# JohannesBuchner/UltraNest

Hardware: AMD Instinct MI355X
Metric: proposal-points filtered/sec (MLFriends.inside) + region-rebuild ms, N=4000 d=50 (higher is better)
Workload: dtype f64; 1 GPU; C5: N=4000 live points, d=50, P=1e6 proposals/step/GPU drawn uniformly inside the wrapping ellipsoid (set E), AffineLayer, 30 bootstraps; one step = MLFriends.inside on a batch resident in HBM; the timed loop visits 3 distinct batches in turn; n_live=4000, d=50, bootstraps=30, parallelism=proposal rows sharded over 1 GPU(s), region replicated

## Files before the change

### ultranest_amd/csrc/mlf_debug.hip

```cpp
#include <hip/hip_runtime.h>

#include <atomic>
#include <vector>

#include "../../include/mlfriends_hip.h"
#include "mlf_host.hpp"
#include "mlf_sample.hpp"

using namespace mlf;

extern "C" {

int mlf_debug_forget_grants(unsigned long long *grants_so_far) {
  if (grants_so_far) *grants_so_far = g_grant_calls.load(std::memory_order_relaxed);
  g_grant_epoch.fetch_add(1u, std::memory_order_acq_rel);
  return 0;
}

int mlf_debug_philox(uint64_t seed, unsigned stream, size_t nblocks, uint32_t *out) {
  if (!out) return fail_arg(MLF_E_BADARG, "null pointer");
  if (nblocks == 0) return 0;
  if (int rc = ensure_ctx()) return rc;
  Ctx &c = g_ctx;
  CK(c.out.reserve(nblocks * 4 * sizeof(unsigned)));
// ... 108 lines not shown
  }
  if (f.segcnt.p && f.segcnt.cap >= sizeof(unsigned)) {
    const size_t n = (size_t)f.last.nsegs;
    std::vector<unsigned> c(n);
    if (n) CK(hipMemcpy(c.data(), f.segcnt.p, n * sizeof(unsigned), hipMemcpyDeviceToHost));
    unsigned long long sum = 0, mx = 0;
    for (unsigned v : c) {
      sum += v;
      mx = v > mx ? v : mx;
    }
    out[2] = sum;
    out[3] = mx;
    out[4] = n;
  }
  if (f.png.p) {
    unsigned g[6];
    CK(hipMemcpy(g, f.png.p, sizeof g, hipMemcpyDeviceToHost));
    out[5] = g[0];
    if (cap > 6) out[6] = g[1];
    if (cap > 7) out[7] = g[5];
  }
  if (cap > 17) {
    out[16] = (unsigned long long)f.last_min.cut[0];
    out[17] = (unsigned long long)f.last_min.cut[1];
  }
  if (cap > 18) out[18] = (f.last_min.defer && (f.last_min.fused_variant & 2u)) ? 1ull : 0ull;
  {
    if (cap >= 16 && f.last.mid && f.last.time_launches && f.segcnt.p) {
      unsigned st[8];
      CK(hipMemcpy(st, f.segcnt.p, sizeof st, hipMemcpyDeviceToHost));
      for (int i = 0; i < 8; ++i) out[8 + i] = st[i];
    } else if (cap >= 16 && f.last.nsegs == uncertain_blocks() && f.segcnt.cap >= (size_t)(f.last.nsegs + 8) * sizeof(unsigned)) {
      unsigned st[8];
      CK(hipMemcpy(st, f.segcnt.as<unsigned>() + uncertain_stamp_base(), sizeof st, hipMemcpyDeviceToHost));
      for (int i = 0; i < 8; ++i) out[8 + i] = st[i];
    }
  }
  return 0;
}
// ... 50 lines not shown
```

### ultranest_amd/csrc/mlf_filter.hpp

```cpp
#pragma once
#include "mlf_common.hpp"
#include "mlf_prep4.hpp"

#define MLF_FILTER_MAXD 128

constexpr int kFilterMaxSplit = 16;

namespace mlf {

struct FilterArgs {
  const void *refF;
  const void *qF;
  const float *tlo, *thi;
  int ntiles32;
  long long ngroups;
  long long nq;
  int *best;
  unsigned long long *list;
  unsigned seg_cap;
  unsigned *seg_count;
  unsigned *counters;
  int tile0, tile1;
  const int *qmap;
  const unsigned *ngroups_dev;
// ... 16 lines not shown
  const void *qF;
  const float *tlo, *thi;
  const int *qmap;
  const int *qmin;
  long long ngroups;
  const unsigned *nslots_dev;
  long long nq;
  int *best;
  void *cq;
  float *ctlo, *cthi;
  int *cmap;
  int *cmin;
  unsigned *ccount;
  unsigned ccap;
  int last;
  unsigned long long *stamps;
  unsigned stamp_block;
};
constexpr unsigned kUncertainListCap = 4096;
struct UncertainArgs {
  const void *refF;
  int ntiles32;
  const void *qF;
  const float *thi;
  const int *qmap;
  const unsigned *nslots_dev;
  const double *pts;
  int d, dp;
  const double *lay_ctr;
  const double *T8;
  int ldt8;
  const double *refR;
  int n;
  double r2;
  int *best;
  unsigned *counters;
  unsigned *seg_count;
  EllExactArgs ell;
  unsigned nsweepblk;
};
hipError_t launch_sweep_min(int ks, int qw, const MinArgs &a, hipStream_t s);
// ... 94 lines not shown
```

### ultranest_amd/csrc/mlf_fused.hip

```cpp
#include "mlf_filter.hpp"
#include "mlf_dpp_dev.hpp"
#include "mlf_filter_dev.hpp"
#include "mlf_prep4.hpp"

#include <math.h>

namespace mlf {

typedef float float16v __attribute__((ext_vector_type(16)));
typedef _Float16 half2v __attribute__((ext_vector_type(2)));
typedef _Float16 half8v __attribute__((ext_vector_type(8)));
typedef float float2v __attribute__((ext_vector_type(2)));
typedef unsigned uint4v __attribute__((ext_vector_type(4)));

#ifndef MLF_OPERAND_STEPS
#define MLF_OPERAND_STEPS 4
#endif
namespace {

template <int DP, int NW = 8>
struct F4 {
  static constexpr int NS = (DP + 15) / 16;
  static constexpr int KS = (DP + 6 + 15) / 16;
  static constexpr int NT = (KS + 1) / 2;
// ... 551 lines not shown
      if ((keepm[g] >> row) & 1u) {
        const unsigned rank = base + (unsigned)__popc(keepm[g] & ((1u << row) - 1u));
        const size_t gd = rank >> 5;
        const unsigned rd = (rank & 31u) + (unsigned)(lane & 32);
        if (rank < a.ccap) {
#pragma unroll
          for (int s = 0; s < KS; ++s) {
            union { half8v h8; uint4 u; } cv;
            cv.h8 = bq[g][s];
            dst[(gd * KS + s) * 64 + rd] = cv.u;
          }
        }
        if (lane < 32 && rank < a.ccap) {
          a.ctlo[rank] = tlo[g];
          a.cthi[rank] = thi[g];
          a.cmap[rank] = (int)((g0 + g) * 32 + p32);
          a.cmin[rank] = qmn[g];
        }
      }
      base += (unsigned)__popc(keepm[g]);
    }
  }
  stamp(12);
}

bool fused_usable(int dp) { return dp >= 2 && dp <= 56 && (dp & 1) == 0; }

template <int D, int NW, bool SQ>
static hipError_t launch_prep_sweep_t(const FusedArgs &a, long long nsets, hipStream_t s) {
  constexpr size_t lds = F4<D, NW>::LDS;
  static_assert(lds <= 160 * 1024 - 64, "LDS budget");
// ... 32 lines not shown
```

### ultranest_amd/csrc/mlf_recheck_dev.hpp

```cpp
#pragma once
#include "mlf_prep4.hpp"

namespace mlf {

constexpr unsigned kEllWaves = 512;

__device__ __forceinline__ void ell_exact_wave(const EllExactArgs &a, double *dls, unsigned wave, unsigned nwaves) {
  const unsigned count = *a.count < a.cap ? *a.count : a.cap;
  const int lane = threadIdx.x & 63;
  const int d = a.d;
  const bool own = lane < d;
  const double *lcol = a.ell_L + (own ? lane : 0);
  const double myctr = own ? a.ell_ctr[lane] : 0.0;
  for (unsigned e = wave; e < count; e += nwaves) {
    const long long p = a.list[e];
    const double *row = a.pts + p * (long long)d;
    const double dl = own ? row[lane] - myctr : 0.0;
    __builtin_amdgcn_wave_barrier();
    dls[lane] = dl;
    __builtin_amdgcn_wave_barrier();
    double y = 0.0;
#pragma unroll 10
    for (int j = 0; j < d; ++j) y = __builtin_fma(lcol[(size_t)j * a.dp], dls[j], y);
    if (!own) y = 0.0;
    double qt = y * y, nrm2 = dl * dl;
    for (int o = 32; o > 0; o >>= 1) {
      qt += __shfl_xor(qt, o, 64);
      nrm2 += __shfl_xor(nrm2, o, 64);
    }
    const double eps = a.eps_scale * nrm2;
    bool inside;
    if (a.chol_ok && qt + eps < a.enlarge) {
      inside = true;
    } else if (a.chol_ok && qt - eps > a.enlarge) {
      inside = false;
    } else {
      double acc = 0.0;
      if (lane == 0) {
        for (int j = 0; j < d; ++j) {
          const double dj = row[j] - a.ell_ctr[j];
          const double *arow = a.ell_A + (size_t)j * a.dp;
          for (int k = 0; k < d; ++k) acc += (dj * arow[k]) * (row[k] - a.ell_ctr[k]);
        }
      }
      acc = __shfl(acc, 0, 64);
      inside = acc <= a.enlarge;
    }
    if (!inside && lane == 0) {
      a.gate[p] = 0;
      if (a.route) a.route[p] = 0;
    }
  }
  if (lane == 0) {
    const unsigned t = atomicAdd(a.done, 1u);
    if (t == nwaves - 1u) {
      if (a.last) *a.last = *a.count;
      *a.count = 0u;
      *a.done = 0u;
    }
  }
}

constexpr int kTQ = 8;
constexpr int kChunk = 32;

// ... 104 lines not shown
```

### ultranest_amd/csrc/mlf_route.hip

```cpp
#include <hip/hip_runtime.h>

#include <algorithm>

#include "../../include/mlfriends_hip.h"
#include "mlf_host.hpp"
#include "mlf_prep3.hpp"
#include "mlf_prep64.hpp"

namespace mlf {

int filter_prepare_refs(FilterCtx &f, const double *refR, int n, int d, int dp, hipStream_t s,
                        bool host_sync) {
  f.refs_ready = false;
  const int ks = (dp + 6 + 15) / 16;
  if (ks > 9 || n < 1 || (long long)round_up(n, 32) / 32 * ks * 1024 >= (1ll << 31)) {
    f.usable = false;
    return 0;
  }
  f.ks = ks;
  const int npad32 = round_up(n, 32);
  f.ntiles32 = npad32 / 32;
  CK(f.stats.reserve((8 + MLF_FILTER_MAXD) * sizeof(double)));
  CK(f.refF.reserve((size_t)npad32 * ks * 16 * 2));
  (void)d;
// ... 86 lines not shown
  if (!p.filter) return p;
  p.ordered = !first_index && f.ordered && opt(f, OPT_ORDER);
  const bool bounded = p.stage == STAGE_PREP4;
  p.mid = bounded && !pregate && !first_index && f.ks <= 4 && mid_usable(r->dp) && nq <= opt(f, OPT_MID_MAX);
  if (p.mid) return p;
  const int want_phases = (int)opt(f, OPT_PHASES);
  const long long phase_min = opt(f, OPT_PHASE_MIN_QUERIES);
  if (want_phases && nq >= phase_min && (phase_min < 32768 || nq * f.ntiles32 >= 30000000ll))
    p.nphase = want_phases >= 2 ? (want_phases <= f.ntiles32 / 4 ? want_phases : (f.ntiles32 >= 16 ? 2 : 1))
                                : (f.ntiles32 >= 16 ? 2 : 1);
  p.narrow = (p.nphase > 1 && f.ks <= 4) ? (int)opt(f, OPT_NARROW_TAIL) : 0;
  const long long ngroups = (nq + 31) / 32;
  p.split = p.nphase == 1 ? filter_tile_split(f.ks, ngroups, f.ntiles32, (int)opt(f, OPT_SPLIT_WAVES)) : 1;
  p.own_recheck = bounded && !first_index && p.nphase == 1;
  p.fold_finish = bounded && p.nphase == 2;
  p.min_path = p.fold_finish && !first_index && f.ks <= 4 && opt(f, OPT_SWEEP_MIN);
  if (p.nphase == 2) {
    const int nt = f.ntiles32, first_pct = (int)opt(f, OPT_FIRST_RANGE_PCT), second_pct = (int)opt(f, OPT_SECOND_RANGE_PCT);
    const int cut = (int)((long long)nt * first_pct / 100);
    p.cut[0] = cut < 4 ? 4 : (cut > nt - 4 ? nt - 4 : cut);
    if (p.min_path && second_pct > 0 && nq * nt >= opt(f, OPT_THIRD_MIN_WORK)) {
      const int cut2 = (int)((long long)nt * second_pct / 100);
      int a = (int)((long long)cut2 * first_pct / 100);
      a = a < 4 ? 4 : a;
      if (cut2 >= a + 4 && cut2 <= nt - 4) {
        p.cut[0] = a;
        p.cut[1] = cut2;
      }
    }
  }
  p.defer = p.min_path && opt(f, OPT_FUSED_FIRST) && fused_usable(r->dp);
// ... 81 lines not shown
  FilterCtx &f = b.f;
  const BatchPlan &p = b.p;
  const ExactSrc &xs = *b.xs;
  const long long nqpad = b.ngroups() * 32;
  const bool min3 = p.cut[1] > 0;
  CK(f.segcnt.reserve((size_t)(p.nsegs + 8) * sizeof(unsigned)));
  CK(f.pmin.reserve((size_t)nqpad * sizeof(int)));
  if (min3) CK(f.pmin2.reserve((size_t)nqpad * sizeof(int)));
  MinArgs m{};
  m.refF = b.opF();
  m.ntiles32 = f.ntiles32;
  m.nq = b.nq;
  m.best = f.best.as<int>();
  m.ngroups = b.ngroups();
  m.ccap = (unsigned)nqpad;
  m.tile0 = 0;
  m.tile1 = p.cut[0];
  m.qF = f.qF.p;
  m.tlo = f.tlo.as<float>();
  m.thi = f.thi.as<float>();
  m.cq = f.pqF[0].p;
  m.ctlo = f.ptlo[0].as<float>();
  m.cthi = f.pthi[0].as<float>();
  m.cmap = f.pmap[0].as<int>();
  m.cmin = f.pmin.as<int>();
  m.ccount = f.png.as<unsigned>() + 2;
  m.last = 0;
  if (p.defer) {
    FusedArgs fu{};
    fu.p = xs.prep;
    fu.refF = b.opF();
    fu.ntiles32 = f.ntiles32;
    fu.tile0 = 0;
    fu.tile1 = p.cut[0];
    fu.cq = m.cq;
    fu.ctlo = m.ctlo;
    fu.cthi = m.cthi;
    fu.cmap = m.cmap;
    fu.cmin = m.cmin;
    fu.ccount = m.ccount;
    fu.ccap = m.ccap;
    if (f.stamp_block >= 0 && f.stamp_block < 1000000) {
// ... 9 lines not shown
  }
  const int usrc = min3 ? 0 : 1;
  m.tile0 = p.cut[0];
  m.tile1 = min3 ? p.cut[1] : f.ntiles32;
  m.qF = f.pqF[0].p;
  m.tlo = f.ptlo[0].as<float>();
  m.thi = f.pthi[0].as<float>();
  m.qmap = f.pmap[0].as<int>();
  m.qmin = f.pmin.as<int>();
  m.nslots_dev = f.png.as<unsigned>() + 2;
  m.cq = f.pqF[1].p;
  m.ctlo = f.ptlo[1].as<float>();
  m.cthi = f.pthi[1].as<float>();
  m.cmap = f.pmap[1].as<int>();
  m.cmin = min3 ? f.pmin2.as<int>() : nullptr;
  m.ccount = f.png.as<unsigned>() + 3;
  m.last = min3 ? 0 : 1;
  auto sweep_stamps = [&](int which) -> int {
    m.stamps = nullptr;
    if (f.stamp_block >= which * 1000000 && f.stamp_block < (which + 1) * 1000000) {
      CK(f.fstamps.reserve(16 * sizeof(unsigned long long)));
      m.stamps = f.fstamps.as<unsigned long long>();
      m.stamp_block = (unsigned)(f.stamp_block - which * 1000000);
    }
    return 0;
  };
  if (int rc = sweep_stamps(1)) return rc;
  if (min3) {
    if (int rc = timed_launch(b, [&] { return launch_sweep_min(f.ks, filter_groups_per_wave(f.ks, 0), m, b.s); })) return rc;
    if (int rc = sweep_stamps(2)) return rc;
    m.tile0 = p.cut[1];
    m.tile1 = f.ntiles32;
    m.qF = f.pqF[1].p;
    m.tlo = f.ptlo[1].as<float>();
    m.thi = f.pthi[1].as<float>();
    m.qmap = f.pmap[1].as<int>();
    m.qmin = f.pmin2.as<int>();
    m.nslots_dev = f.png.as<unsigned>() + 3;
    m.cq = f.pqF[0].p;
    m.ctlo = f.ptlo[0].as<float>();
    m.cthi = f.pthi[0].as<float>();
    m.cmap = f.pmap[0].as<int>();
    m.cmin = nullptr;
    m.ccount = f.png.as<unsigned>() + 4;
    m.last = 1;
  }
  if (int rc = timed_launch(b, [&] { return launch_sweep_min(f.ks, filter_groups_per_wave(f.ks, 0), m, b.s); })) return rc;
  UncertainArgs ua{};
  ua.refF = b.opF();
  ua.ntiles32 = f.ntiles32;
  ua.qF = f.pqF[usrc].p;
  ua.thi = f.pthi[usrc].as<float>();
  ua.qmap = f.pmap[usrc].as<int>();
  ua.nslots_dev = f.png.as<unsigned>() + (min3 ? 4 : 3);
  ua.pts = xs.pts;
  ua.d = b.L.d;
  ua.dp = b.L.dp;
  ua.lay_ctr = xs.lay_ctr;
  ua.T8 = xs.T8;
  ua.ldt8 = xs.ldt;
  ua.refR = b.opR();
  ua.n = b.L.n;
  ua.r2 = b.L.r2;
  ua.best = f.best.as<int>();
  ua.counters = f.counters.as<unsigned>();
  ua.seg_count = f.segcnt.as<unsigned>();
  ua.ell = xs.ell;
  if (int rc = timed_launch(b, [&] { return launch_uncertain(f.ks, ua, b.s); })) return rc;
  if (b.ev_after) CK(hipEventRecord(b.ev_after, b.s));
// ... 120 lines not shown
  const int mode = b.out_idx ? SCAN_FIRST : SCAN_MASK;
  if (!b.xs)
    launch_filter_finalize(f.route.as<uint8_t>(), f.best.as<int>(), f.counters.as<unsigned>(), b.nq, b.out_mask,
                           b.out_idx, f.gate2.as<uint8_t>(), b.s);
  ScanArgs a = b.xs ? scan_args(b.L, b.xs->pts, b.L.d, 1, b.nq, mode) : scan_args(b.L, b.q, b.ldq, b.ldk, b.nq, mode);
  a.gate = f.gate2.as<uint8_t>();
  a.out_idx = b.out_idx;
  a.out_mask = b.out_mask;
  a.only_gated = 1;
  if (b.xs) {
    scan_finalise(a, f, *b.xs);
    a.fin_best = f.best.as<int>();
    if (p.fold_finish) {
      a.fin_slots = f.png.as<unsigned>() + 2;
      a.fin_groups = f.png.as<unsigned>();
      if (p.min_path) a.fin_slots2 = f.png.as<unsigned>() + (p.cut[1] > 0 ? 4 : 3);
      if (p.cut[1] > 0) a.fin_slots3 = f.png.as<unsigned>() + 3;
    }
  }
  CK(launch_scan(b.L.dp, a, b.s));
  CK(hipGetLastError());
  return 0;
}

}

int filter_run(const FilterBatch &b) {
  FilterCtx &f = b.f;
  const BatchPlan &p = b.p;
  const long long nqpad = b.ngroups() * 32;
  f.last = p;
  if (p.min_path) f.last_min = p;
  if (int rc = filter_reserve(f, p, b.nq)) return rc;
  if (p.stage != STAGE_PREP4 && p.stage != STAGE_PREP3)
    launch_quant_queries(b.q, b.ldq, b.nq, nqpad, b.L.d, b.L.dp, f.ks, f.stats.as<double>(), b.L.r2, b.gate, f.qF.p,
                         f.tlo.as<float>(), f.thi.as<float>(), f.route.as<uint8_t>(), f.best.as<int>(),
                         f.counters.as<unsigned>(), b.s);
  CK(hipGetLastError());
  if (p.nphase > 1) {
    for (int i = 0; i < 2; ++i) {
      CK(f.pqF[i].reserve((size_t)nqpad * f.ks * 16 * 2));
      CK(f.ptlo[i].reserve((size_t)nqpad * sizeof(float)));
      CK(f.pthi[i].reserve((size_t)nqpad * sizeof(float)));
      CK(f.pmap[i].reserve((size_t)nqpad * sizeof(int)));
    }
    if (!f.png.p) {
      CK(f.png.reserve(8 * sizeof(unsigned)));
      CK(hipMemset(f.png.p, 0, 8 * sizeof(unsigned)));
    } else if (f.png_dirty) {
      CK(hipMemsetAsync(f.png.p, 0, 8 * sizeof(unsigned), b.s));
    }
    f.png_dirty = true;
  }
  if (int rc = p.min_path ? filter_sweep_min(b) : filter_phases(b)) return rc;
  if (!p.min_path && !p.own_recheck)
    if (int rc = filter_recheck(b)) return rc;
  if (int rc = filter_scan_tail(b)) return rc;
  if (p.nphase > 1) f.png_dirty = false;
  return 0;
}

}
```

### ultranest_amd/csrc/mlf_scan.hip

```cpp
#include "mlf_common.hpp"

namespace mlf {

template <int DP, int QB, bool EXTRA>
__global__ __launch_bounds__(kScanThreads) void k_scan(ScanArgs a) {
  constexpr int kScanQB = QB;
  __shared__ __attribute__((aligned(16))) double qs[kScanQB * DP];
  __shared__ int state[kScanQB];
  __shared__ int cnt[kScanQB];

  const int tid = threadIdx.x;
  const int lane = tid & 63;
  const int wave = tid >> 6;
  __shared__ int any_active;
  if (EXTRA && a.fin_best && blockIdx.x >= a.fin_grid0) {
    const long long p0 = (((long long)blockIdx.x - a.fin_grid0) * kScanThreads + tid) * 4;
    if (p0 == 0 && a.fin_reset) *a.fin_reset = 0u;
    if (p0 == 0 && a.fin_slots) {
      *a.fin_groups = (*a.fin_slots + 31u) / 32u;
      *a.fin_slots = 0u;
    }
    if (p0 == 0 && a.fin_slots2) {
      a.fin_groups[1] = *a.fin_slots2;
      *a.fin_slots2 = 0u;
    }
    if (p0 == 0 && a.fin_slots3) {
      a.fin_groups[5] = (*a.fin_slots3 + 31u) / 32u;
      *a.fin_slots3 = 0u;
    } else if (p0 == 0 && a.fin_slots2) {
      a.fin_groups[5] = 0u;
    }
    if (p0 >= a.nq) return;
    const bool overflowed = a.counters[1] != 0u;
    int rt[4], b[4];
    if (p0 + 3 < a.nq) {
      const uchar4 r4 = *reinterpret_cast<const uchar4 *>(a.route + p0);
      const int4 b4 = *reinterpret_cast<const int4 *>(a.fin_best + p0);
      rt[0] = r4.x, rt[1] = r4.y, rt[2] = r4.z, rt[3] = r4.w;
      b[0] = b4.x, b[1] = b4.y, b[2] = b4.z, b[3] = b4.w;
// ... 190 lines not shown
```

### ultranest_amd/csrc/mlf_sweepmin.hip

```cpp
#include "mlf_filter.hpp"
#include "mlf_dpp_dev.hpp"
#include "mlf_filter_dev.hpp"
#include "mlf_recheck_dev.hpp"

#include <math.h>

namespace mlf {

typedef __attribute__((ext_vector_type(8))) _Float16 half8;
typedef __attribute__((ext_vector_type(16))) float float16v;
typedef __attribute__((ext_vector_type(4))) unsigned uint4v;

namespace {

__device__ __forceinline__ int min3i(int a, int b, int c) {
  const int m = a < b ? a : b;
  return m < c ? m : c;
}

constexpr int kPosInf = 0x7f800000;

template <int KS>
__device__ __forceinline__ void load_tile(half8 (&A)[KS], __amdgpu_buffer_rsrc_t rsrc, int voff, int soff) {
#pragma unroll
// ... 37 lines not shown

constexpr int min_waves(int ks, int qw, int pf) {
  const int need = 16 * qw + 4 * ks * qw + 4 * ks * (pf + 1) + 40;
  return (qw <= 2 && ks * qw <= 8) ? 4 : (need <= 128 ? 4 : (need <= 168 ? 3 : 2));
}

constexpr long long kSweepMinSetGrid = 1024;

}

template <int KS, int QW, int PF>
__global__ __launch_bounds__(256) __attribute__((amdgpu_waves_per_eu(min_waves(KS, QW, PF)))) void k_sweep_min(MinArgs a) {
  const int lane = threadIdx.x & 63;
  const long long nslots = a.nslots_dev ? (long long)*a.nslots_dev : -1;
  const long long ngroups = nslots >= 0 ? (nslots + 31) / 32 : a.ngroups;
  __shared__ unsigned wg_keep[4], wg_base;
  bool stamp_on = a.stamps != nullptr && blockIdx.x == a.stamp_block && threadIdx.x < 64;
  auto stamp = [&](int k) __attribute__((always_inline)) {
    if (stamp_on) {
      const unsigned long long t = __builtin_readcyclecounter();
      if (lane == 0) a.stamps[k] = t;
    }
  };
  stamp(0);
  auto stamp_rt = [&](int k) __attribute__((always_inline)) {
    if (a.stamps != nullptr && threadIdx.x == 0) {
      if (blockIdx.x == 0) a.stamps[8 + k] = __builtin_amdgcn_s_memrealtime();
      if (blockIdx.x == a.stamp_block) a.stamps[10 + k] = __builtin_amdgcn_s_memrealtime();
    }
  };
  stamp_rt(0);
  for (unsigned bidx = blockIdx.x, pass = 0;; bidx += gridDim.x, ++pass) {
  if ((long long)bidx * (4 * QW) >= ngroups) break;
  if (pass) __syncthreads();
  const long long wave = (long long)bidx * 4 + (threadIdx.x >> 6);
  const long long g0 = wave * QW;
  if (g0 >= ngroups) {
    if (lane == 0) wg_keep[threadIdx.x >> 6] = 0u;
    __syncthreads();
    __syncthreads();
    continue;
  }

  const half8 *qF = reinterpret_cast<const half8 *>(a.qF);
  half8 bq[QW][KS];
  float tlo[QW], thi[QW];
  int run[QW], qnum[QW];
#pragma unroll
  for (int g = 0; g < QW; ++g) {
    const long long grp = (g0 + g < ngroups) ? g0 + g : ngroups - 1;
#pragma unroll
    for (int s = 0; s < KS; ++s) bq[g][s] = qF[((size_t)grp * KS + s) * 64 + lane];
    const long long qi = grp * 32 + (lane & 31);
    const bool have = g0 + g < ngroups && (nslots < 0 || qi < nslots);
    tlo[g] = have ? a.tlo[qi] : -1.0f;
    thi[g] = have ? a.thi[qi] : -1.0f;
    if (!have) {
#pragma unroll
      for (int s = 0; s < KS; ++s) bq[g][s] = (half8){0, 0, 0, 0, 0, 0, 0, 0};
    }
    run[g] = (a.qmin && have && lane < 32) ? a.qmin[qi] : kPosInf;
    qnum[g] = have ? (a.qmap ? a.qmap[qi] : (int)qi) : -1;
  }

  const int ntl = a.tile1 - a.tile0;
  const int tstart = a.tile0 + (int)(((long long)bidx * 37) % ntl);
  constexpr int kTileBytes = KS * 1024;
  const __amdgpu_buffer_rsrc_t rsrc =
      __builtin_amdgcn_make_buffer_rsrc(const_cast<void *>(a.refF), 0, a.ntiles32 * kTileBytes, 0x00020000);
  const int voff = lane * 16;
  const int off_begin = a.tile0 * kTileBytes, off_end = a.tile1 * kTileBytes;

  float16v acc[QW];
  auto mm = [&](const half8(&A)[KS], int ga, int gb) __attribute__((always_inline)) {
#pragma unroll
    for (int s = 0; s < KS; ++s) {
// ... 47 lines not shown
  } else {
    int off = tstart * kTileBytes;
    load_tile<KS>(A0, rsrc, voff, off);
    for (int it = 0; it < ntl; it += 2) {
      const int offn = next_off(off);
      load_tile<KS>(A1, rsrc, voff, offn);
      tile(A0);
      if (it + 1 >= ntl) break;
      off = next_off(offn);
      load_tile<KS>(A0, rsrc, voff, off);
      tile(A1);
    }
  }

  stamp(3);
  unsigned keepm[QW];
  int qid[QW], qmn[QW];
#pragma unroll
  for (int g = 0; g < QW; ++g) {
    keepm[g] = 0u;
    qid[g] = -1;
    qmn[g] = kPosInf;
    if (g0 + g >= ngroups) continue;
    const long long qi = qnum[g];
    const int m = half_min32(run[g]);
    const float mf = __int_as_float(m);
    const bool valid = qi >= 0 && qi < a.nq && thi[g] > 0.0f;
    const bool hit = valid && mf <= tlo[g];
    if (lane < 32 && hit) a.best[qi] = 0;
    const bool keep = valid && !hit && (a.last ? mf <= thi[g] : true);
    keepm[g] = (unsigned)__ballot(keep);
    qid[g] = (int)qi;
    qmn[g] = m;
  }
  unsigned total = 0;
#pragma unroll
  for (int g = 0; g < QW; ++g) total += (unsigned)__popc(keepm[g]);
  if (lane == 0) wg_keep[threadIdx.x >> 6] = total;
  stamp(4);
  __syncthreads();
  stamp(5);
  if (threadIdx.x == 0) {
    const unsigned all = wg_keep[0] + wg_keep[1] + wg_keep[2] + wg_keep[3];
    wg_base = all ? atomicAdd(a.ccount, all) : 0u;
  }
  __syncthreads();
  stamp(6);
  if (total != 0u) {
    unsigned base = wg_base;
    for (int w = 0; w < (int)(threadIdx.x >> 6); ++w) base += wg_keep[w];
    base = (unsigned)__builtin_amdgcn_readfirstlane((int)base);
    uint4 *dst = reinterpret_cast<uint4 *>(a.cq);
    const unsigned row = (unsigned)(lane & 31);
#pragma unroll
    for (int g = 0; g < QW; ++g) {
      if ((keepm[g] >> row) & 1u) {
        const unsigned rank = base + (unsigned)__popc(keepm[g] & ((1u << row) - 1u));
        const size_t gd = rank >> 5;
        const unsigned rd = (rank & 31u) + (unsigned)(lane & 32);
        if (rank < a.ccap) {
#pragma unroll
          for (int s = 0; s < KS; ++s) {
            union { half8 h; uint4 u; } cv;
            cv.h = bq[g][s];
            dst[(gd * KS + s) * 64 + rd] = cv.u;
          }
        }
        if (lane < 32 && rank < a.ccap) {
          a.ctlo[rank] = tlo[g];
          a.cthi[rank] = thi[g];
          a.cmap[rank] = qid[g];
          if (a.cmin) a.cmin[rank] = qmn[g];
        }
      }
      base += (unsigned)__popc(keepm[g]);
    }
  }
  stamp(7);
  if (stamp_on || (pass == 0 && blockIdx.x == 0)) stamp_rt(1);
  stamp_on = false;
  }
}

template <class T>
using lds_t = __attribute__((address_space(3))) T;
template <class T>
__device__ __forceinline__ lds_t<T> *lds_ptr(T *p) {
  return (lds_t<T> *)p;
}
template <class T>
__device__ __forceinline__ const lds_t<T> *lds_ptr(const T *p) {
  return (const lds_t<T> *)p;
}

template <int KS>
__device__ __attribute__((noinline)) void uncertain_sweep(const void *refF_, int ntiles32_, const void *qF_, const float *thi_, long long set_,
                                                          long long ngroups_, long long nslots_, unsigned *plist_, unsigned *lcount_,
                                                          int wv_, int lane) {
  constexpr int QW = 4;
  lds_t<unsigned> *plist = lds_ptr(plist_);
  lds_t<unsigned> *lcount = lds_ptr(lcount_);
  const void *refF = uni(refF_);
  const int ntiles32 = uni(ntiles32_), wv = uni(wv_);
  const long long set = uni(set_), ngroups = uni(ngroups_), nslots = uni(nslots_);
  qF_ = uni(qF_);
  thi_ = uni(thi_);
  typedef __attribute__((address_space(1))) const half8 ghalf8;
  typedef __attribute__((address_space(1))) const float gfloat;
  ghalf8 *qF = (ghalf8 *)qF_;
  gfloat *thig = (gfloat *)thi_;
  constexpr int kTileBytes = KS * 1024;
  const __amdgpu_buffer_rsrc_t rsrc =
      __builtin_amdgcn_make_buffer_rsrc(const_cast<void *>(refF), 0, ntiles32 * kTileBytes, 0x00020000);
  const int voff = lane * 16;
  const int rowbase = 4 * (lane >> 5);
  const long long g0 = set * QW;
  half8 bq[QW][KS];
  float thi[QW];
#pragma unroll
  for (int g = 0; g < QW; ++g) {
    const long long grp = (g0 + g < ngroups) ? g0 + g : ngroups - 1;
#pragma unroll
    for (int s = 0; s < KS; ++s) bq[g][s] = qF[((size_t)grp * KS + s) * 64 + lane];
    const long long qi = grp * 32 + (lane & 31);
    const bool have = g0 + g < ngroups && qi < nslots;
    thi[g] = have ? thig[qi] : -1.0f;
    if (!have) {
#pragma unroll
      for (int s = 0; s < KS; ++s) bq[g][s] = (half8){0, 0, 0, 0, 0, 0, 0, 0};
    }
  }
  const int tile0 = ntiles32 * wv / 8, tile1 = ntiles32 * (wv + 1) / 8;
  __builtin_amdgcn_s_waitcnt(0x0F70);
  float16v acc[QW];
  auto mm = [&](const half8(&A)[KS], int ga, int gb) __attribute__((always_inline)) {
#pragma unroll
    for (int s = 0; s < KS; ++s) {
      const float16v z = {0.f, 0.f, 0.f, 0.f, 0.f, 0.f, 0.f, 0.f, 0.f, 0.f, 0.f, 0.f, 0.f, 0.f, 0.f, 0.f};
      acc[ga] = __builtin_amdgcn_mfma_f32_32x32x16_f16(A[s], bq[ga][s], s == 0 ? z : acc[ga], 0, 0, 0);
      acc[gb] = __builtin_amdgcn_mfma_f32_32x32x16_f16(A[s], bq[gb][s], s == 0 ? z : acc[gb], 0, 0, 0);
    }
  };
  auto list_group = [&](int g, int t) __attribute__((always_inline)) {
    const float16v &c = acc[g];
    const int tm = tree_min(c, kPosInf);
    const bool flagged = __int_as_float(tm) <= thi[g];
    if (__ballot(flagged) == 0ull) return;
// ... 110 lines not shown
    for (int ct = 0; ct < NC; ++ct) t[ct] = __builtin_amdgcn_mfma_f64_16x16x4f64(afr[ct], bfr[ks], t[ct], 0, 0, 0);
  }
  __builtin_amdgcn_wave_barrier();
  lds_t<double> *out = tq + (16 * wv + q) * ds;
#pragma unroll
  for (int ct = 0; ct < NC; ++ct)
#pragma unroll
    for (int r = 0; r < 4; ++r) {
      const int c = 16 * ct + kq + 4 * r;
      if (c < d) out[c] = t[ct][r];
    }
}

template <int KS, int NCH>
__global__ __launch_bounds__(512, 1) void k_uncertain(UncertainArgs a) {
  constexpr int QW = 4;
  extern __shared__ __attribute__((aligned(16))) double lds_u[];
  const int lane = threadIdx.x & 63, wv = threadIdx.x >> 6;
  const int d = a.d, ds = uncertain_row_stride(d);
  double *tq = lds_u;
  double *tl = tq + 128 * ds;
  unsigned *plist = reinterpret_cast<unsigned *>(tl + a.dp * a.ldt8);
  int *qid = reinterpret_cast<int *>(plist + kUncertainListCap);
  unsigned *lcount = reinterpret_cast<unsigned *>(qid + 128);
  const unsigned nsweepblk = a.nsweepblk;
  if (blockIdx.x >= nsweepblk) {
    if (a.ell.count) ell_exact_wave(a.ell, lds_u + wv * 64, (blockIdx.x - nsweepblk) * 8 + wv, (gridDim.x - nsweepblk) * 8);
    return;
  }
  if (blockIdx.x == 0 && threadIdx.x == 0) {
#pragma unroll
    for (int k = 0; k < 8; ++k) a.seg_count[uncertain_stamp_base() + k] = 0u;
  }
  const long long nslots = (long long)*a.nslots_dev;
  if ((long long)blockIdx.x * 128 >= nslots) {
    if (threadIdx.x == 0) a.seg_count[blockIdx.x] = 0u;
    return;
  }
  unsigned nstamp = 0u;
  auto stamp = [&]() __attribute__((always_inline)) {
    if (blockIdx.x == 0 && threadIdx.x == 0 && nstamp < 8u) a.seg_count[uncertain_stamp_base() + nstamp] = (unsigned)__builtin_readcyclecounter();
    ++nstamp;
  };
  stamp();
  {
    double v[8];
    const int nt = a.dp * a.ldt8;
#pragma unroll
    for (int it = 0; it < 8; ++it) v[it] = threadIdx.x + it * 512 < nt ? a.T8[threadIdx.x + it * 512] : 0.0;
#pragma unroll
    for (int it = 0; it < 8; ++it)
      if (threadIdx.x + it * 512 < nt) tl[threadIdx.x + it * 512] = v[it];
  }
  const long long ngroups = (nslots + 31) / 32;
  const long long nsets = (ngroups + QW - 1) / QW;
  unsigned listed_total = 0u;

  for (long long set = blockIdx.x; set < nsets; set += nsweepblk) {
    __syncthreads();
    if (threadIdx.x == 0) *lcount = 0u;
    if (threadIdx.x < 128) {
      const long long slot = set * 128 + threadIdx.x;
      qid[threadIdx.x] = slot < nslots ? a.qmap[slot] : -1;
    }
    __syncthreads();
    stamp();
    uncertain_sweep<KS>(a.refF, a.ntiles32, a.qF, a.thi, set, ngroups, nslots, plist, lcount, wv, lane);
    stamp();
    {
      double v[16];
#pragma unroll
      for (int it = 0; it < 16; ++it) {
        const int e = threadIdx.x + it * 512;
        const int ql = e / d, k = e - ql * d;
        const int q = e < 128 * d ? qid[ql] : -1;
        v[it] = q >= 0 ? a.pts[(long long)q * d + k] - a.lay_ctr[k] : 0.0;
      }
#pragma unroll
      for (int it = 0; it < 16; ++it) {
        const int e = threadIdx.x + it * 512;
        const int ql = e / d, k = e - ql * d;
        if (e < 128 * d) tq[ql * ds + k] = v[it];
// ... 78 lines not shown
```

### ultranest_amd/kernels.py

```python
import ctypes

import numpy as np

from . import _lib
from ._lib import check, f64, ptr

int_dtype = np.int64


def find_nearby(apts, bpts, radiussq, nnearby):
    apts, bpts = f64(apts), f64(bpts)
    if apts.ndim != 2 or bpts.ndim != 2:
        raise ValueError("apts and bpts must be 2-d")
    nb = bpts.shape[0]
    d = bpts.shape[1] if nb else apts.shape[1]
    if nb and apts.shape[0] and apts.shape[1] != bpts.shape[1]:
        raise ValueError("dimensionality mismatch")
    if nnearby.dtype != int_dtype or nnearby.ndim != 1 or len(nnearby) != nb:
        raise ValueError("nnearby must be an int64 vector of len(bpts)")
    out = nnearby if nnearby.flags.c_contiguous else np.empty(nb, dtype=int_dtype)
    check(_lib.lib().mlf_find_nearby(ptr(apts), apts.shape[0], ptr(bpts), nb, d, float(radiussq), ptr(out)))
    if out is not nnearby:
        nnearby[:] = out

# ... 333 lines not shown
        check(_lib.lib().mlf_region_timing_filter_launches(self._h, ctypes.byref(n), ctypes.byref(ms)))
        return n.value, ms.value

    def timing_filter_launch_ms(self, cap=4096):
        ms = np.empty(cap)
        n = ctypes.c_int(0)
        check(_lib.lib().mlf_region_timing_filter_launch_ms(self._h, ptr(ms), cap, ctypes.byref(n)))
        return ms[:min(n.value, cap)].copy()

    def filter_info(self, npts):
        act, k, t = ctypes.c_int(0), ctypes.c_int(0), ctypes.c_int(0)
        check(_lib.lib().mlf_region_filter_info(self._h, int(npts), ctypes.byref(act), ctypes.byref(k), ctypes.byref(t)))
        return bool(act.value), k.value, t.value

    def debug_stats(self):
        out = np.zeros(19, dtype=np.uint64)
        check(_lib.lib().mlf_region_debug_stats(self._h, ptr(out), 19))
        keys = ("ellipsoid_band", None, "uncertain_pairs", "largest_segment", "segments", "second_range_groups",
                "uncertain_queries", "third_range_groups")
        stats = {k: int(v) for k, v in zip(keys, out[:8]) if k}
        stats["range_cuts"] = [int(out[16]), int(out[17])]
        stats["same_quadratic_form"] = int(out[18])
        if out[8]:
            st = out[8:16].astype(np.int64)
            stats["uncertain_stage_cycles"] = [int((st[i + 1] - st[i]) & 0xffffffff) for i in range(6) if st[i + 1]]
            stats["stamp7"] = int(st[7])
        return stats

    def fused_stamps(self, block):
        out = np.zeros(16, dtype=np.uint64)
        check(_lib.lib().mlf_region_debug_fused_stamps(self._h, -1 if block is None else int(block), ptr(out), 16))
        st = out[:16].astype(np.int64)
        return [int(x - st[0]) if x else None for x in st] if st[0] else None

    def time_inside_dev(self, d_pts, npts, d_mask, stream=0, reps=3):
        tot, scan = ctypes.c_float(0), ctypes.c_float(0)
        check(_lib.lib().mlf_region_time_inside_dev(self._h, ctypes.c_void_p(d_pts), npts, ctypes.c_void_p(d_mask),
# ... 16 lines not shown
```

Before: 2.920 billion proposals/s.

## Split uncertain query lists by tile range and batch ellipsoid exact checks

The last sweep-min pass now sorts each surviving query into per-range lists, using flags that record which tile ranges could still hold a match. The uncertain kernel then sweeps each query only over the tile range it was flagged for, instead of over all tiles. Separately, the exact ellipsoid recheck handles four points per wave to increase memory-level parallelism. The cost is more complex bookkeeping: list capacity is split evenly across ranges with an overflow flag, and there are extra atomics and ballots per group.

```diff
diff --git a/ultranest_amd/csrc/mlf_debug.hip b/ultranest_amd/csrc/mlf_debug.hip
--- a/ultranest_amd/csrc/mlf_debug.hip
+++ b/ultranest_amd/csrc/mlf_debug.hip
@@ -146,8 +146,10 @@
     out[4] = n;
   }
   if (f.png.p) {
-    unsigned g[6];
+    unsigned g[16];
     CK(hipMemcpy(g, f.png.p, sizeof g, hipMemcpyDeviceToHost));
+    if (cap > 21)
+      for (int l = 0; l < 3; ++l) out[19 + l] = g[12 + l];
     out[5] = g[0];
     if (cap > 6) out[6] = g[1];
     if (cap > 7) out[7] = g[5];
@@ -155,6 +157,11 @@
   if (cap > 17) {
     out[16] = (unsigned long long)f.last_min.cut[0];
     out[17] = (unsigned long long)f.last_min.cut[1];
+  }
+  if (cap > 22 && f.counters.p) {
+    unsigned c[2];
+    CK(hipMemcpy(c, f.counters.p, sizeof c, hipMemcpyDeviceToHost));
+    out[22] = c[1];
   }
   if (cap > 18) out[18] = (f.last_min.defer && (f.last_min.fused_variant & 2u)) ? 1ull : 0ull;
   {
diff --git a/ultranest_amd/csrc/mlf_filter.hpp b/ultranest_amd/csrc/mlf_filter.hpp
--- a/ultranest_amd/csrc/mlf_filter.hpp
+++ b/ultranest_amd/csrc/mlf_filter.hpp
@@ -54,9 +54,15 @@
   unsigned *ccount;
   unsigned ccap;
   int last;
+  int range;
+  unsigned share;
+  unsigned *counters;
   unsigned long long *stamps;
   unsigned stamp_block;
 };
+constexpr int kRangeFlagShift = 28;
+constexpr int kRangeQueryMask = (1 << kRangeFlagShift) - 1;
+constexpr int kMaxRanges = 3;
 constexpr unsigned kUncertainListCap = 4096;
 struct UncertainArgs {
   const void *refF;
@@ -65,6 +71,9 @@
   const float *thi;
   const int *qmap;
   const unsigned *nslots_dev;
+  int nlists;
+  unsigned share;
+  int cut[kMaxRanges + 1];
   const double *pts;
   int d, dp;
   const double *lay_ctr;
diff --git a/ultranest_amd/csrc/mlf_fused.hip b/ultranest_amd/csrc/mlf_fused.hip
--- a/ultranest_amd/csrc/mlf_fused.hip
+++ b/ultranest_amd/csrc/mlf_fused.hip
@@ -589,7 +589,7 @@
         if (lane < 32 && rank < a.ccap) {
           a.ctlo[rank] = tlo[g];
           a.cthi[rank] = thi[g];
-          a.cmap[rank] = (int)((g0 + g) * 32 + p32);
+          a.cmap[rank] = (int)((g0 + g) * 32 + p32) | ((__int_as_float(qmn[g]) <= thi[g] ? 1 : 0) << kRangeFlagShift);
           a.cmin[rank] = qmn[g];
         }
       }
diff --git a/ultranest_amd/csrc/mlf_recheck_dev.hpp b/ultranest_amd/csrc/mlf_recheck_dev.hpp
--- a/ultranest_amd/csrc/mlf_recheck_dev.hpp
+++ b/ultranest_amd/csrc/mlf_recheck_dev.hpp
@@ -5,6 +5,7 @@
 
 constexpr unsigned kEllWaves = 512;
 
+template <int NI = 1>
 __device__ __forceinline__ void ell_exact_wave(const EllExactArgs &a, double *dls, unsigned wave, unsigned nwaves) {
   const unsigned count = *a.count < a.cap ? *a.count : a.cap;
   const int lane = threadIdx.x & 63;
@@ -12,43 +13,63 @@
   const bool own = lane < d;
   const double *lcol = a.ell_L + (own ? lane : 0);
   const double myctr = own ? a.ell_ctr[lane] : 0.0;
-  for (unsigned e = wave; e < count; e += nwaves) {
-    const long long p = a.list[e];
-    const double *row = a.pts + p * (long long)d;
-    const double dl = own ? row[lane] - myctr : 0.0;
+  for (unsigned e0 = wave; e0 < count; e0 += NI * nwaves) {
+    long long p[NI];
+    const double *row[NI];
+    double dl[NI], y[NI];
+    bool on[NI];
+#pragma unroll
+    for (int i = 0; i < NI; ++i) {
+      const unsigned e = e0 + (unsigned)i * nwaves;
+      on[i] = e < count;
+      p[i] = a.list[on[i] ? e : e0];
+      row[i] = a.pts + p[i] * (long long)d;
+    }
+#pragma unroll
+    for (int i = 0; i < NI; ++i) dl[i] = own ? row[i][lane] - myctr : 0.0;
     __builtin_amdgcn_wave_barrier();
-    dls[lane] = dl;
+#pragma unroll
+    for (int i = 0; i < NI; ++i) dls[i * 64 + lane] = dl[i];
     __builtin_amdgcn_wave_barrier();
-    double y = 0.0;
+#pragma unroll
+    for (int i = 0; i < NI; ++i) y[i] = 0.0;
 #pragma unroll 10
-    for (int j = 0; j < d; ++j) y = __builtin_fma(lcol[(size_t)j * a.dp], dls[j], y);
-    if (!own) y = 0.0;
-    double qt = y * y, nrm2 = dl * dl;
-    for (int o = 32; o > 0; o >>= 1) {
-      qt += __shfl_xor(qt, o, 64);
-      nrm2 += __shfl_xor(nrm2, o, 64);
+    for (int j = 0; j < d; ++j) {
+      const double lj = lcol[(size_t)j * a.dp];
+#pragma unroll
+      for (int i = 0; i < NI; ++i) y[i] = __builtin_fma(lj, dls[i * 64 + j], y[i]);
     }
-    const double eps = a.eps_scale * nrm2;
-    bool inside;
-    if (a.chol_ok && qt + eps < a.enlarge) {
-      inside = true;
-    } else if (a.chol_ok && qt - eps > a.enlarge) {
-      inside = false;
-    } else {
-      double acc = 0.0;
-      if (lane == 0) {
-        for (int j = 0; j < d; ++j) {
-          const double dj = row[j] - a.ell_ctr[j];
-          const double *arow = a.ell_A + (size_t)j * a.dp;
-          for (int k = 0; k < d; ++k) acc += (dj * arow[k]) * (row[k] - a.ell_ctr[k]);
+#pragma unroll
+    for (int i = 0; i < NI; ++i) {
+      if (!on[i]) continue;
+      const double yi = own ? y[i] : 0.0;
+      double qt = yi * yi, nrm2 = dl[i] * dl[i];
+      for (int o = 32; o > 0; o >>= 1) {
+        qt += __shfl_xor(qt, o, 64);
+        nrm2 += __shfl_xor(nrm2, o, 64);
+      }
+      const double eps = a.eps_scale * nrm2;
+      bool inside;
+      if (a.chol_ok && qt + eps < a.enlarge) {
+        inside = true;
+      } else if (a.chol_ok && qt - eps > a.enlarge) {
+        inside = false;
+      } else {
+        double acc = 0.0;
+        if (lane == 0) {
+          for (int j = 0; j < d; ++j) {
+            const double dj = row[i][j] - a.ell_ctr[j];
+            const double *arow = a.ell_A + (size_t)j * a.dp;
+            for (int k = 0; k < d; ++k) acc += (dj * arow[k]) * (row[i][k] - a.ell_ctr[k]);
+          }
         }
+        acc = __shfl(acc, 0, 64);
+        inside = acc <= a.enlarge;
       }
-      acc = __shfl(acc, 0, 64);
-      inside = acc <= a.enlarge;
-    }
-    if (!inside && lane == 0) {
-      a.gate[p] = 0;
-      if (a.route) a.route[p] = 0;
+      if (!inside && lane == 0) {
+        a.gate[p[i]] = 0;
+        if (a.route) a.route[p[i]] = 0;
+      }
     }
   }
   if (lane == 0) {
diff --git a/ultranest_amd/csrc/mlf_route.hip b/ultranest_amd/csrc/mlf_route.hip
--- a/ultranest_amd/csrc/mlf_route.hip
+++ b/ultranest_amd/csrc/mlf_route.hip
@@ -124,7 +124,7 @@
   p.split = p.nphase == 1 ? filter_tile_split(f.ks, ngroups, f.ntiles32, (int)opt(f, OPT_SPLIT_WAVES)) : 1;
   p.own_recheck = bounded && !first_index && p.nphase == 1;
   p.fold_finish = bounded && p.nphase == 2;
-  p.min_path = p.fold_finish && !first_index && f.ks <= 4 && opt(f, OPT_SWEEP_MIN);
+  p.min_path = p.fold_finish && !first_index && f.ks <= 4 && opt(f, OPT_SWEEP_MIN) && nq <= kRangeQueryMask;
   if (p.nphase == 2) {
     const int nt = f.ntiles32, first_pct = (int)opt(f, OPT_FIRST_RANGE_PCT), second_pct = (int)opt(f, OPT_SECOND_RANGE_PCT);
     const int cut = (int)((long long)nt * first_pct / 100);
@@ -236,6 +236,10 @@
   m.best = f.best.as<int>();
   m.ngroups = b.ngroups();
   m.ccap = (unsigned)nqpad;
+  m.counters = f.counters.as<unsigned>();
+  const int nlists = min3 ? 3 : 2;
+  const unsigned share = (unsigned)round_up((int)((nqpad + nlists - 1) / nlists), 128);
+  unsigned *const list_counters = f.png.as<unsigned>() + 8;
   m.tile0 = 0;
   m.tile1 = p.cut[0];
   m.qF = f.qF.p;
@@ -248,6 +252,7 @@
   m.cmin = f.pmin.as<int>();
   m.ccount = f.png.as<unsigned>() + 2;
   m.last = 0;
+  m.range = 0;
   if (p.defer) {
     FusedArgs fu{};
     fu.p = xs.prep;
@@ -287,8 +292,10 @@
   m.cthi = f.pthi[1].as<float>();
   m.cmap = f.pmap[1].as<int>();
   m.cmin = min3 ? f.pmin2.as<int>() : nullptr;
-  m.ccount = f.png.as<unsigned>() + 3;
+  m.ccount = min3 ? f.png.as<unsigned>() + 3 : list_counters;
   m.last = min3 ? 0 : 1;
+  m.range = 1;
+  m.share = share;
   auto sweep_stamps = [&](int which) -> int {
     m.stamps = nullptr;
     if (f.stamp_block >= which * 1000000 && f.stamp_block < (which + 1) * 1000000) {
@@ -315,8 +322,9 @@
     m.cthi = f.pthi[0].as<float>();
     m.cmap = f.pmap[0].as<int>();
     m.cmin = nullptr;
-    m.ccount = f.png.as<unsigned>() + 4;
+    m.ccount = list_counters;
     m.last = 1;
+    m.range = 2;
   }
   if (int rc = timed_launch(b, [&] { return launch_sweep_min(f.ks, filter_groups_per_wave(f.ks, 0), m, b.s); })) return rc;
   UncertainArgs ua{};
@@ -325,7 +333,13 @@
   ua.qF = f.pqF[usrc].p;
   ua.thi = f.pthi[usrc].as<float>();
   ua.qmap = f.pmap[usrc].as<int>();
-  ua.nslots_dev = f.png.as<unsigned>() + (min3 ? 4 : 3);
+  ua.nslots_dev = list_counters;
+  ua.nlists = nlists;
+  ua.share = share;
+  ua.cut[0] = 0;
+  ua.cut[1] = p.cut[0];
+  ua.cut[2] = min3 ? p.cut[1] : f.ntiles32;
+  ua.cut[3] = f.ntiles32;
   ua.pts = xs.pts;
   ua.d = b.L.d;
   ua.dp = b.L.dp;
@@ -476,7 +490,7 @@
     if (p.fold_finish) {
       a.fin_slots = f.png.as<unsigned>() + 2;
       a.fin_groups = f.png.as<unsigned>();
-      if (p.min_path) a.fin_slots2 = f.png.as<unsigned>() + (p.cut[1] > 0 ? 4 : 3);
+      if (p.min_path) a.fin_slots2 = f.png.as<unsigned>() + 8;
       if (p.cut[1] > 0) a.fin_slots3 = f.png.as<unsigned>() + 3;
     }
   }
@@ -500,17 +514,18 @@
                          f.counters.as<unsigned>(), b.s);
   CK(hipGetLastError());
   if (p.nphase > 1) {
+    const size_t nslot = (size_t)nqpad + kMaxRanges * 128;
     for (int i = 0; i < 2; ++i) {
-      CK(f.pqF[i].reserve((size_t)nqpad * f.ks * 16 * 2));
-      CK(f.ptlo[i].reserve((size_t)nqpad * sizeof(float)));
-      CK(f.pthi[i].reserve((size_t)nqpad * sizeof(float)));
-      CK(f.pmap[i].reserve((size_t)nqpad * sizeof(int)));
+      CK(f.pqF[i].reserve(nslot * f.ks * 16 * 2));
+      CK(f.ptlo[i].reserve(nslot * sizeof(float)));
+      CK(f.pthi[i].reserve(nslot * sizeof(float)));
+      CK(f.pmap[i].reserve(nslot * sizeof(int)));
     }
     if (!f.png.p) {
-      CK(f.png.reserve(8 * sizeof(unsigned)));
-      CK(hipMemset(f.png.p, 0, 8 * sizeof(unsigned)));
+      CK(f.png.reserve(16 * sizeof(unsigned)));
+      CK(hipMemset(f.png.p, 0, 16 * sizeof(unsigned)));
     } else if (f.png_dirty) {
-      CK(hipMemsetAsync(f.png.p, 0, 8 * sizeof(unsigned), b.s));
+      CK(hipMemsetAsync(f.png.p, 0, 16 * sizeof(unsigned), b.s));
     }
     f.png_dirty = true;
   }
diff --git a/ultranest_amd/csrc/mlf_scan.hip b/ultranest_amd/csrc/mlf_scan.hip
--- a/ultranest_amd/csrc/mlf_scan.hip
+++ b/ultranest_amd/csrc/mlf_scan.hip
@@ -21,8 +21,12 @@
       *a.fin_slots = 0u;
     }
     if (p0 == 0 && a.fin_slots2) {
-      a.fin_groups[1] = *a.fin_slots2;
-      *a.fin_slots2 = 0u;
+      const uint4 c = *reinterpret_cast<const uint4 *>(a.fin_slots2);
+      a.fin_groups[1] = c.w;
+      a.fin_groups[12] = c.x;
+      a.fin_groups[13] = c.y;
+      a.fin_groups[14] = c.z;
+      *reinterpret_cast<uint4 *>(a.fin_slots2) = make_uint4(0u, 0u, 0u, 0u);
     }
     if (p0 == 0 && a.fin_slots3) {
       a.fin_groups[5] = (*a.fin_slots3 + 31u) / 32u;
diff --git a/ultranest_amd/csrc/mlf_sweepmin.hip b/ultranest_amd/csrc/mlf_sweepmin.hip
--- a/ultranest_amd/csrc/mlf_sweepmin.hip
+++ b/ultranest_amd/csrc/mlf_sweepmin.hip
@@ -75,7 +75,7 @@
   const int lane = threadIdx.x & 63;
   const long long nslots = a.nslots_dev ? (long long)*a.nslots_dev : -1;
   const long long ngroups = nslots >= 0 ? (nslots + 31) / 32 : a.ngroups;
-  __shared__ unsigned wg_keep[4], wg_base;
+  __shared__ __attribute__((aligned(16))) unsigned wg_keep[4][4], wg_base[4];
   bool stamp_on = a.stamps != nullptr && blockIdx.x == a.stamp_block && threadIdx.x < 64;
   auto stamp = [&](int k) __attribute__((always_inline)) {
     if (stamp_on) {
@@ -97,7 +97,7 @@
   const long long wave = (long long)bidx * 4 + (threadIdx.x >> 6);
   const long long g0 = wave * QW;
   if (g0 >= ngroups) {
-    if (lane == 0) wg_keep[threadIdx.x >> 6] = 0u;
+    if (lane < 4) wg_keep[threadIdx.x >> 6][lane] = 0u;
     __syncthreads();
     __syncthreads();
     continue;
@@ -106,7 +106,7 @@
   const half8 *qF = reinterpret_cast<const half8 *>(a.qF);
   half8 bq[QW][KS];
   float tlo[QW], thi[QW];
-  int run[QW], qnum[QW];
+  int run[QW], car[QW], qnum[QW];
 #pragma unroll
   for (int g = 0; g < QW; ++g) {
     const long long grp = (g0 + g < ngroups) ? g0 + g : ngroups - 1;
@@ -120,7 +120,8 @@
 #pragma unroll
       for (int s = 0; s < KS; ++s) bq[g][s] = (half8){0, 0, 0, 0, 0, 0, 0, 0};
     }
-    run[g] = (a.qmin && have && lane < 32) ? a.qmin[qi] : kPosInf;
+    run[g] = kPosInf;
+    car[g] = (a.qmin && have) ? a.qmin[qi] : kPosInf;
     qnum[g] = have ? (a.qmap ? a.qmap[qi] : (int)qi) : -1;
   }
 
@@ -198,66 +199,100 @@
   }
 
   stamp(3);
-  unsigned keepm[QW];
   int qid[QW], qmn[QW];
+  unsigned fl[QW], km[QW][kMaxRanges];
+  unsigned tot[4] = {0u, 0u, 0u, 0u};
 #pragma unroll
   for (int g = 0; g < QW; ++g) {
-    keepm[g] = 0u;
+    fl[g] = 0u;
     qid[g] = -1;
     qmn[g] = kPosInf;
+#pragma unroll
+    for (int l = 0; l < kMaxRanges; ++l) km[g][l] = 0u;
     if (g0 + g >= ngroups) continue;
-    const long long qi = qnum[g];
-    const int m = half_min32(run[g]);
+    const long long qi = qnum[g] < 0 ? -1ll : (long long)(qnum[g] & kRangeQueryMask);
+    const int own = half_min32(run[g]);
+    const int m = own < car[g] ? own : car[g];
     const float mf = __int_as_float(m);
     const bool valid = qi >= 0 && qi < a.nq && thi[g] > 0.0f;
     const bool hit = valid && mf <= tlo[g];
     if (lane < 32 && hit) a.best[qi] = 0;
     const bool keep = valid && !hit && (a.last ? mf <= thi[g] : true);
-    keepm[g] = (unsigned)__ballot(keep);
-    qid[g] = (int)qi;
+    unsigned flags = (qnum[g] < 0 ? 0u : (unsigned)qnum[g] >> kRangeFlagShift) | ((__int_as_float(own) <= thi[g] ? 1u : 0u) << a.range);
+    fl[g] = keep ? (a.last ? (flags ? flags : 1u << a.range) : 1u) : 0u;
+    qid[g] = (int)qi | (int)(flags << kRangeFlagShift);
     qmn[g] = m;
-  }
-  unsigned total = 0;
-#pragma unroll
-  for (int g = 0; g < QW; ++g) total += (unsigned)__popc(keepm[g]);
-  if (lane == 0) wg_keep[threadIdx.x >> 6] = total;
+#pragma unroll
+    for (int l = 0; l < kMaxRanges; ++l) {
+      km[g][l] = (unsigned)__ballot((fl[g] >> l) & 1u);
+      tot[l] += (unsigned)__popc(km[g][l]);
+    }
+    tot[3] += (unsigned)__popc((unsigned)__ballot(keep));
+  }
+  if (lane < 4) wg_keep[threadIdx.x >> 6][lane] = lane == 0 ? tot[0] : (lane == 1 ? tot[1] : (lane == 2 ? tot[2] : tot[3]));
   stamp(4);
   __syncthreads();
   stamp(5);
-  if (threadIdx.x == 0) {
-    const unsigned all = wg_keep[0] + wg_keep[1] + wg_keep[2] + wg_keep[3];
-    wg_base = all ? atomicAdd(a.ccount, all) : 0u;
+  if (threadIdx.x < 4 && (threadIdx.x == 0 || a.last)) {
+    const int l = (int)threadIdx.x;
+    const unsigned all = wg_keep[0][l] + wg_keep[1][l] + wg_keep[2][l] + wg_keep[3][l];
+    wg_base[l] = all ? atomicAdd(a.ccount + l, all) : 0u;
   }
   __syncthreads();
   stamp(6);
-  if (total != 0u) {
-    unsigned base = wg_base;
-    for (int w = 0; w < (int)(threadIdx.x >> 6); ++w) base += wg_keep[w];
-    base = (unsigned)__builtin_amdgcn_readfirstlane((int)base);
+  if (tot[3] != 0u) {
+    const unsigned cap = a.last ? a.share : a.ccap;
+    const unsigned share = a.last ? a.share : 0u;
+    const int wv = (int)(threadIdx.x >> 6);
+    unsigned base[kMaxRanges];
+    {
+      const uint4 b4 = *reinterpret_cast<const uint4 *>(wg_base);
+      const uint4 k0 = *reinterpret_cast<const uint4 *>(wg_keep[0]), k1 = *reinterpret_cast<const uint4 *>(wg_keep[1]),
+                  k2 = *reinterpret_cast<const uint4 *>(wg_keep[2]);
+      base[0] = b4.x + (wv > 0 ? k0.x : 0u) + (wv > 1 ? k1.x : 0u) + (wv > 2 ? k2.x : 0u);
+      base[1] = b4.y + (wv > 0 ? k0.y : 0u) + (wv > 1 ? k1.y : 0u) + (wv > 2 ? k2.y : 0u);
+      base[2] = b4.z + (wv > 0 ? k0.z : 0u) + (wv > 1 ? k1.z : 0u) + (wv > 2 ? k2.z : 0u);
+#pragma unroll
+      for (int l = 0; l < kMaxRanges; ++l) base[l] = (unsigned)__builtin_amdgcn_readfirstlane((int)base[l]);
+    }
     uint4 *dst = reinterpret_cast<uint4 *>(a.cq);
-    const unsigned row = (unsigned)(lane & 31);
+    const unsigned below = (1u << (lane & 31)) - 1u;
 #pragma unroll
     for (int g = 0; g < QW; ++g) {
-      if ((keepm[g] >> row) & 1u) {
-        const unsigned rank = base + (unsigned)__popc(keepm[g] & ((1u << row) - 1u));
-        const size_t gd = rank >> 5;
-        const unsigned rd = (rank & 31u) + (unsigned)(lane & 32);
-        if (rank < a.ccap) {
-#pragma unroll
-          for (int s = 0; s < KS; ++s) {
-            union { half8 h; uint4 u; } cv;
-            cv.h = bq[g][s];
-            dst[(gd * KS + s) * 64 + rd] = cv.u;
+      if ((km[g][0] | km[g][1] | km[g][2]) == 0u) continue;
+      unsigned rank[kMaxRanges];
+#pragma unroll
+      for (int l = 0; l < kMaxRanges; ++l) {
+        rank[l] = base[l] + (unsigned)__popc(km[g][l] & below);
+        base[l] += (unsigned)__popc(km[g][l]);
+      }
+      unsigned rem = fl[g];
+      do {
+        if (rem != 0u) {
+          const unsigned l = (unsigned)__builtin_ctz(rem);
+          const unsigned rk = l == 0u ? rank[0] : (l == 1u ? rank[1] : rank[2]);
+          const unsigned slot = l * share + rk;
+          const size_t gd = slot >> 5;
+          const unsigned rd = (slot & 31u) + (unsigned)(lane & 32);
+          if (rk < cap) {
+#pragma unroll
+            for (int s = 0; s < KS; ++s) {
+              union { half8 h; uint4 u; } cv;
+              cv.h = bq[g][s];
+              dst[(gd * KS + s) * 64 + rd] = cv.u;
+            }
+            if (lane < 32) {
+              a.ctlo[slot] = tlo[g];
+              a.cthi[slot] = thi[g];
+              a.cmap[slot] = qid[g];
+              if (a.cmin) a.cmin[slot] = qmn[g];
+            }
+          } else if (a.last && lane < 32) {
+            a.counters[1] = 1u;
           }
+          rem &= rem - 1u;
         }
-        if (lane < 32 && rank < a.ccap) {
-          a.ctlo[rank] = tlo[g];
-          a.cthi[rank] = thi[g];
-          a.cmap[rank] = qid[g];
-          if (a.cmin) a.cmin[rank] = qmn[g];
-        }
-      }
-      base += (unsigned)__popc(keepm[g]);
+      } while (__ballot(rem != 0u) != 0ull);
     }
   }
   stamp(7);
@@ -278,14 +313,14 @@
 }
 
 template <int KS>
-__device__ __attribute__((noinline)) void uncertain_sweep(const void *refF_, int ntiles32_, const void *qF_, const float *thi_, long long set_,
-                                                          long long ngroups_, long long nslots_, unsigned *plist_, unsigned *lcount_,
-                                                          int wv_, int lane) {
+__device__ __attribute__((noinline)) void uncertain_sweep(const void *refF_, int ntiles32_, int rtile0_, int rtile1_, const void *qF_,
+                                                          const float *thi_, long long set_, long long ngroups_, long long nslots_,
+                                                          unsigned *plist_, unsigned *lcount_, int wv_, int lane) {
   constexpr int QW = 4;
   lds_t<unsigned> *plist = lds_ptr(plist_);
   lds_t<unsigned> *lcount = lds_ptr(lcount_);
   const void *refF = uni(refF_);
-  const int ntiles32 = uni(ntiles32_), wv = uni(wv_);
+  const int ntiles32 = uni(ntiles32_), wv = uni(wv_), rtile0 = uni(rtile0_), rtile1 = uni(rtile1_);
   const long long set = uni(set_), ngroups = uni(ngroups_), nslots = uni(nslots_);
   qF_ = uni(qF_);
   thi_ = uni(thi_);
@@ -314,7 +349,7 @@
       for (int s = 0; s < KS; ++s) bq[g][s] = (half8){0, 0, 0, 0, 0, 0, 0, 0};
     }
   }
-  const int tile0 = ntiles32 * wv / 8, tile1 = ntiles32 * (wv + 1) / 8;
+  const int tile0 = rtile0 + (rtile1 - rtile0) * wv / 8, tile1 = rtile0 + (rtile1 - rtile0) * (wv + 1) / 8;
   __builtin_amdgcn_s_waitcnt(0x0F70);
   float16v acc[QW];
   auto mm = [&](const half8(&A)[KS], int ga, int gb) __attribute__((always_inline)) {
@@ -455,7 +490,6 @@
 
 template <int KS, int NCH>
 __global__ __launch_bounds__(512, 1) void k_uncertain(UncertainArgs a) {
-  constexpr int QW = 4;
   extern __shared__ __attribute__((aligned(16))) double lds_u[];
   const int lane = threadIdx.x & 63, wv = threadIdx.x >> 6;
   const int d = a.d, ds = uncertain_row_stride(d);
@@ -466,17 +500,12 @@
   unsigned *lcount = reinterpret_cast<unsigned *>(qid + 128);
   const unsigned nsweepblk = a.nsweepblk;
   if (blockIdx.x >= nsweepblk) {
-    if (a.ell.count) ell_exact_wave(a.ell, lds_u + wv * 64, (blockIdx.x - nsweepblk) * 8 + wv, (gridDim.x - nsweepblk) * 8);
+    if (a.ell.count) ell_exact_wave<4>(a.ell, lds_u + wv * 256, (blockIdx.x - nsweepblk) * 8 + wv, (gridDim.x - nsweepblk) * 8);
     return;
   }
   if (blockIdx.x == 0 && threadIdx.x == 0) {
 #pragma unroll
     for (int k = 0; k < 8; ++k) a.seg_count[uncertain_stamp_base() + k] = 0u;
-  }
-  const long long nslots = (long long)*a.nslots_dev;
-  if ((long long)blockIdx.x * 128 >= nslots) {
-    if (threadIdx.x == 0) a.seg_count[blockIdx.x] = 0u;
-    return;
   }
   unsigned nstamp = 0u;
   auto stamp = [&]() __attribute__((always_inline)) {
@@ -484,29 +513,59 @@
     ++nstamp;
   };
   stamp();
-  {
-    double v[8];
-    const int nt = a.dp * a.ldt8;
-#pragma unroll
-    for (int it = 0; it < 8; ++it) v[it] = threadIdx.x + it * 512 < nt ? a.T8[threadIdx.x + it * 512] : 0.0;
-#pragma unroll
-    for (int it = 0; it < 8; ++it)
-      if (threadIdx.x + it * 512 < nt) tl[threadIdx.x + it * 512] = v[it];
-  }
-  const long long ngroups = (nslots + 31) / 32;
-  const long long nsets = (ngroups + QW - 1) / QW;
+  double tv[8];
+  const int nt = a.dp * a.ldt8;
+#pragma unroll
+  for (int it = 0; it < 8; ++it) tv[it] = threadIdx.x + it * 512 < nt ? a.T8[threadIdx.x + it * 512] : 0.0;
+  unsigned cnt[kMaxRanges], nsets[kMaxRanges], nwork = 0u;
+#pragma unroll
+  for (int l = 0; l < kMaxRanges; ++l) {
+    const unsigned c = l < a.nlists ? a.nslots_dev[l] : 0u;
+    cnt[l] = c < a.share ? c : a.share;
+    nsets[l] = (cnt[l] + 127u) / 128u;
+    nwork += nsets[l];
+  }
+  if (blockIdx.x >= nwork) {
+    if (threadIdx.x == 0) a.seg_count[blockIdx.x] = 0u;
+    return;
+  }
+  auto locate = [&](unsigned w, int &l, long long &slot0, long long &slot1) __attribute__((always_inline)) {
+    l = a.nlists - 1;
+#pragma unroll
+    for (int k = kMaxRanges - 1; k > 0; --k)
+      if (k < a.nlists && l == k && w >= nsets[k]) {
+        w -= nsets[k];
+        l = k - 1;
+      }
+    slot0 = (long long)l * a.share + (long long)w * 128;
+    slot1 = (long long)l * a.share + (l == 0 ? cnt[0] : (l == 1 ? cnt[1] : cnt[2]));
+  };
+  int qfirst = -1;
+  if (threadIdx.x < 128) {
+    int l;
+    long long slot0, slot1;
+    locate(blockIdx.x, l, slot0, slot1);
+    qfirst = slot0 + threadIdx.x < slot1 ? (a.qmap[slot0 + threadIdx.x] & kRangeQueryMask) : -1;
+  }
+#pragma unroll
+  for (int it = 0; it < 8; ++it)
+    if (threadIdx.x + it * 512 < nt) tl[threadIdx.x + it * 512] = tv[it];
   unsigned listed_total = 0u;
 
-  for (long long set = blockIdx.x; set < nsets; set += nsweepblk) {
+  for (unsigned w = blockIdx.x; w < nwork; w += nsweepblk) {
+    int l;
+    long long slot0, slot1;
+    locate(w, l, slot0, slot1);
+    const long long set = slot0 / 128, nslots = slot1, ngroups = (slot1 + 31) / 32;
     __syncthreads();
     if (threadIdx.x == 0) *lcount = 0u;
     if (threadIdx.x < 128) {
-      const long long slot = set * 128 + threadIdx.x;
-      qid[threadIdx.x] = slot < nslots ? a.qmap[slot] : -1;
+      const long long slot = slot0 + threadIdx.x;
+      qid[threadIdx.x] = w == blockIdx.x ? qfirst : (slot < nslots ? (a.qmap[slot] & kRangeQueryMask) : -1);
     }
     __syncthreads();
     stamp();
-    uncertain_sweep<KS>(a.refF, a.ntiles32, a.qF, a.thi, set, ngroups, nslots, plist, lcount, wv, lane);
+    uncertain_sweep<KS>(a.refF, a.ntiles32, a.cut[l], a.cut[l + 1], a.qF, a.thi, set, ngroups, nslots, plist, lcount, wv, lane);
     stamp();
     {
       double v[16];
diff --git a/ultranest_amd/kernels.py b/ultranest_amd/kernels.py
--- a/ultranest_amd/kernels.py
+++ b/ultranest_amd/kernels.py
@@ -371,13 +371,15 @@
         return bool(act.value), k.value, t.value
 
     def debug_stats(self):
-        out = np.zeros(19, dtype=np.uint64)
-        check(_lib.lib().mlf_region_debug_stats(self._h, ptr(out), 19))
+        out = np.zeros(23, dtype=np.uint64)
+        check(_lib.lib().mlf_region_debug_stats(self._h, ptr(out), 23))
         keys = ("ellipsoid_band", None, "uncertain_pairs", "largest_segment", "segments", "second_range_groups",
                 "uncertain_queries", "third_range_groups")
         stats = {k: int(v) for k, v in zip(keys, out[:8]) if k}
         stats["range_cuts"] = [int(out[16]), int(out[17])]
         stats["same_quadratic_form"] = int(out[18])
+        stats["uncertain_by_range"] = [int(v) for v in out[19:22]]
+        stats["list_overflow"] = int(out[22])
         if out[8]:
             st = out[8:16].astype(np.int64)
             stats["uncertain_stage_cycles"] = [int((st[i + 1] - st[i]) & 0xffffffff) for i in range(6) if st[i + 1]]
```

Result: no change. 2.923 billion proposals/s, median of 2 (+0.1%).
